# leonsick/depthg

Hardware: AMD Instinct MI355X
Metric: correlation-loss steps/sec at B=32,C=384,28x28 (fwd+bwd, per-GPU batch 32) (higher is better)
Workload: dtype bf16 (feats) / f16 (code) MFMA inputs, f32 accumulate

## Files before the change

### depthg_amd/_lib.py

```python
import ctypes
import os

_HERE = os.path.dirname(os.path.abspath(__file__))
LIB_PATH = os.environ.get("DEPTHG_LIB") or os.path.join(_HERE, "lib", "libdepthg_hip.so")

DG_OUT_COUNT = 9
DG_OUT_TOTAL = 8
DG_VERSION = 118
DG_POINTWISE, DG_ZERO_CLAMP, DG_STABALIZE, DG_DEPTH_TERM, DG_NEED_GRAD, DG_SHARED_COORDS, DG_IDENTITY_GRID, DG_LINE_GRID, \
    DG_EXACT_MASKS, DG_FEATS_UNIT = (1 << i for i in range(10))
DG_LIN_LAYERNORM, DG_LIN_GELU, DG_LIN_IN_BF16, DG_LIN_OUT_BF16 = 1, 2, 4, 8

class CorrDesc(ctypes.Structure):
    _fields_ = [("B", ctypes.c_int32), ("C", ctypes.c_int32), ("D", ctypes.c_int32), ("h", ctypes.c_int32),
                ("w", ctypes.c_int32), ("S", ctypes.c_int32), ("n_neg", ctypes.c_int32),
                ("depth_h", ctypes.c_int32), ("depth_w", ctypes.c_int32), ("flags", ctypes.c_uint32),
                ("shift_intra", ctypes.c_float), ("shift_inter", ctypes.c_float), ("shift_neg", ctypes.c_float),
                ("shift_depth", ctypes.c_float),
                ("w_intra", ctypes.c_float), ("w_inter", ctypes.c_float), ("w_neg", ctypes.c_float),
                ("w_depth", ctypes.c_float), ("code_h", ctypes.c_int32), ("code_w", ctypes.c_int32)]


class AdamSeg(ctypes.Structure):
    _fields_ = [("param", ctypes.c_void_p), ("grad", ctypes.c_void_p), ("exp_avg", ctypes.c_void_p), ("exp_avg_sq", ctypes.c_void_p),
# ... 64 lines not shown
    "dg_crfloss_forward": (_I, [vp, vp] + [i32] * 7 + [vp, i32] + [f32] * 6 + [vp, _SZ, vp, vp]),
    "dg_crfloss_backward": (_I, [vp, _SZ, vp] + [i32] * 6 + [vp, vp, vp]),
    "dg_augalign_workspace_bytes": (_SZ, [i32] * 5),
    "dg_augalign_forward": (_I, [vp] * 3 + [i32] * 7 + [vp, _SZ, vp, vp]),
    "dg_augalign_backward": (_I, [vp, vp, vp, _SZ] + [i32] * 5 + [vp] * 4),
    "dg_recloss_workspace_bytes": (_SZ, [i32] * 5),
    "dg_recloss_forward": (_I, [vp] * 5 + [f32] + [i32] * 5 + [vp, _SZ, vp, vp]),
    "dg_recloss_backward": (_I, [vp] * 5 + [f32, vp, _SZ] + [i32] * 5 + [vp] * 5),
    "dg_adam_step": (_I, [ctypes.POINTER(AdamSeg), i32, ctypes.POINTER(AdamGroup), i32, i32, vp, vp]),
    "dg_attention_workspace_bytes": (_SZ, [i32] * 3),
    "dg_attention_forward": (_I, [vp] + [i32] * 4 + [f32, vp, vp, _SZ, vp]),
    "dg_vit_linear_packed_bytes": (_SZ, [i32] * 2),
    "dg_vit_linear_pack": (_I, [vp, i32, i32, vp, vp]),
    "dg_vit_linear_forward": (_I, [vp, vp, vp, f32, vp, vp, vp, vp] + [i32] * 4 + [vp]),
    "dg_corr_main_kernel_name": (_STR, [cp]),
    "dg_corr_intra_folded": (_I, [cp]),
    "dg_prof_main_span": (_I, [vp]),
    "dg_corr_relaunch_main": (_I, [cp, vp, vp, _SZ, vp]),
}
EXPORTS = list(SIGNATURES)

_lib = None


def load():
    global _lib
    if _lib is not None:
        return _lib
    if not os.path.exists(LIB_PATH):
        raise RuntimeError(
# ... 19 lines not shown
```

### depthg_amd/csrc/dg_api_corr.hip

```cpp
#include "dg_api.h"
#include "dg_corr_args.h"
#include "dg_taps.h"

static unsigned long long* g_prof_span = nullptr;
extern "C" int dg_prof_main_span(void* span) { g_prof_span = static_cast<unsigned long long*>(span); return DG_OK; }

enum class Prep { Small, Dense, General };
enum class Sampler { Plane, ChannelLast };
enum class MainKernel { Small, Corr2, CorrMain };
enum class Depth { None, Job, GsBlocks, GsOwnLaunch };
enum class Hist { Rows, Blobs };
enum class Masks { None, Sampled, DenseRaw, DenseSplit };

struct PairSet {
    int op;
    int neg;
    bool mapped;
    float shift;
    int slot_loss, slot_cd;
    float fin_scale;
    int gidx, csel, dest;
    float factor;
};
struct Operand {
// ... 1 lines not shown
    int cset;
    int map;
};

struct Plan {
    int B, C, D, h, w, hc, wc, S, Sh, P, Ppad, KF, KD, C4, D4, N, T, nops, rf, nrb;
    bool shared, depth, grad, pointwise;
    Prep prep;
    Sampler sampler;
    MainKernel main;
    Masks masks;
    Hist hist;
    bool fold;
    bool half;
    Depth depth_run;
    int nsplit;
    int dep_nrb;
    float lo, hi;
    float shift_depth;
    float inv_numel;
    float grad_f, grad_fn;
    int blob, blob_off_c;
    PairSet ps[DG_MAX_NEG + 2];
    Operand ops[DG_MAX_NEG + 2];
    bool gr_on;
    int gr_nkeys, gr_cpb, gr_blocks_per_image;
    int8_t gr_key[DG_MAX_JOBS], gr_first[DG_MAX_JOBS];
    int32_t gr_nblk[DG_MAX_JOBS];
    size_t nhwc_f[2], nhwc_c[2];
    size_t rows_f[DG_MAX_NEG + 2], rows_c[DG_MAX_NEG + 2];
// ... 147 lines not shown
    p.ticket = take(256);
    const bool xmask = rows && !p.small() && p.grad && plain_zero_clamp && p.Ppad <= 256 && p.rf == 4;
    const bool xmask_dense = (d->flags & DG_EXACT_MASKS) && ident && p.grad && plain_zero_clamp &&
                             p.KF == 384 && p.KD == 96 && p.D <= 80 && p.Ppad >= 160 && p.B <= 64;
    if ((d->flags & DG_EXACT_MASKS) && p.grad && (d->flags & DG_ZERO_CLAMP) && !xmask && !xmask_dense && !p.small())
        return fail(DG_ERR_UNSUPPORTED, "DG_EXACT_MASKS: exact clamp masks exist on small sample grids (always on there) and on the dense "
                                        "identity grid with C <= 384 (padded to 384), D <= 80, P >= 160, B <= 64, zero_clamp without stabalize");
    p.masks = xmask ? Masks::Sampled : (!xmask_dense ? Masks::None : (p.pointwise ? Masks::DenseSplit : Masks::DenseRaw));
    for (int t = 0; t < p.T; ++t) p.maskbits[t] = take(p.has_masks() ? B * (size_t)(p.Ppad / 32) * p.Ppad * 4 : 0);
    p.main = p.small() ? MainKernel::Small
                       : (p.grad && dg_corr2_shape_supported(p.KF, p.KD, p.D, p.lo, p.hi, p.Ppad, p.B) ? MainKernel::Corr2 : MainKernel::CorrMain);
    static const bool fold_on = [] { const char* e = getenv("DG_FOLD_INTRA"); return !(e && e[0] == '0'); }();
    p.fold = fold_on && p.main == MainKernel::Corr2 && p.pointwise && !xmask;
    p.half = p.main == MainKernel::Corr2 && ident && p.N * p.B <= 512 && p.S == p.h && p.S == p.w;
    p.depth_run = (!p.depth || p.small()) ? Depth::None : (!p.grad ? Depth::Job : (p.dense_masks() ? Depth::GsOwnLaunch : Depth::GsBlocks));
    for (int i = 0; i < 2; ++i) p.clo[i] = take(p.masks == Masks::DenseSplit ? B * (size_t)(p.Ppad / 32) * p.KD * 64 : 0);
    p.gr_list = take((size_t)DG_MAX_JOBS * B * DG_GR_CAP * 4);
    p.gr_count = take((size_t)DG_MAX_JOBS * B * 4);
    p.gr_rank = take((size_t)DG_MAX_JOBS * B * 2);
    {
        const bool sg = p.small() && p.grad, two = sg && p.pointwise;
        const size_t gt = B * p.Ppad * p.KD * 4;
        for (int t = 0; t < p.T; ++t) {
            p.dRA2[t] = take(two ? gt : 0);
            p.dRBs[t] = take(sg && p.nsplit == 2 ? gt : 0);
            for (int k = 0; k < 2; ++k) p.dRB2[t][k] = take(two && k < p.nsplit ? gt : 0);
            p.dRBm[t] = take(sg && t >= 2 && (p.pointwise || p.nsplit == 2) ? gt : 0);
        }
        p.part4 = take(p.small() ? (size_t)(p.T + 1) * B * p.nsplit * 16 : 0);
        p.om = take(p.small() ? (size_t)(p.T + 1) * 4 : 0);
// ... 311 lines not shown
        f.ext_inv = c.feat_inv ? c.feat_inv + (size_t)o * p.B * p.P : nullptr;
        f.K = p.C; f.K4 = p.C4; f.Kpad = p.KF; f.is_code = 0; f.h = p.h; f.w = p.w;
        DgGatherJob& k = g.jobs[nj++];
        k.src = p.plane() ? f32(c.ws, p.rows_c[o]) : f32(c.ws, p.nhwc_c[srcsel]); k.coords = c.coords(o); k.srcidx = idx;
        k.blob = c.ws + p.op[o]; k.inv_norm = f32(c.ws, p.inv[o]); k.colpart = f32(c.ws, p.ccolpart[o]);
        k.K = p.D; k.K4 = p.D4; k.Kpad = p.KD; k.is_code = 1; k.h = p.hc; k.w = p.wc;
    }
    g.njobs = nj;
    g.direct = p.plane() ? 1 : 0;
    if (p.masks == Masks::Sampled) cd_mask_args(c, p.rows_c, g.cd);
    g.pre = pre_late;
    DG_HIP(dg_launch_gather(g, p.KF, c.stream));
    return DG_OK;
}

static int fwd_colmeans(Fwd& c) {
    const Plan& p = c.p;
    const DgCorrArgs& a = c.a;
    DgColmeanArgs m;
    memset(&m, 0, sizeof(m));
    m.nops = p.nops; m.B = p.B; m.P = p.P; m.Ppad = p.Ppad; m.KF = p.KF; m.KD = p.KD;
    for (int o = 0; o < p.nops; ++o) {
        m.colpart[o] = p.pointwise ? f32(c.ws, p.colpart[o]) : nullptr; m.bbar[o] = f32(c.ws, p.bbar[o]);
        m.bsplit[o] = reinterpret_cast<__bf16*>(c.ws + p.bsplit[o]);
        m.ngroups[o] = p.Ppad / 32;
        m.ccolpart[o] = f32(c.ws, p.ccolpart[o]); m.csum[o] = f32(c.ws, p.csum[o]);
    }
    m.zero_word = p.depth_in_gs() ? reinterpret_cast<unsigned int*>(c.ws + p.ticket) : nullptr;
    m.zero_words9 = a.wctr;
    if (p.gr_on) {
        m.gr.nh = p.T; m.gr.nkeys = p.gr_nkeys; m.gr.B = p.B;
        for (int t = 0; t < p.T; ++t) { m.gr.sidx[t] = p.map_of(t, c.perms); m.gr.key[t] = p.gr_key[t]; }
        m.gr.list = reinterpret_cast<int32_t*>(c.ws + p.gr_list); m.gr.count = reinterpret_cast<int32_t*>(c.ws + p.gr_count);
        m.gr.rank = reinterpret_cast<int16_t*>(c.ws + p.gr_rank);
    }
    if (p.dense() && p.pointwise) {
        m.dc.code[0] = c.code; m.dc.code[1] = c.code_pos;
        for (int o = 0; o < 2; ++o) { m.dc.blob[o] = c.ws + p.op[o]; m.dc.inv_norm[o] = f32(c.ws, p.inv[o]); m.dc.ccolpart[o] = f32(c.ws, p.ccolpart[o]); }
        m.dc.B = p.B; m.dc.D = p.D; m.dc.KF = p.KF; m.dc.KD = p.KD; m.dc.h = p.h; m.dc.w = p.w; m.dc.P = p.P; m.dc.Ppad = p.Ppad;
        if (p.masks == Masks::DenseSplit) { m.dc.clo[0] = c.ws + p.clo[0]; m.dc.clo[1] = c.ws + p.clo[1]; }
    }
    if (c.split) {
        DgColmeanArgs ms = m;
        ms.zsel = 1; m.zsel = 2;
        DG_HIP(c.side->hand_over(0));
        DG_HIP(dg_launch_colmean(ms, c.side->stream()));
    }
    DG_HIP(dg_launch_colmean(m, c.stream));
    return DG_OK;
}

static int fwd_cd_mask3(Fwd& c) {
    const Plan& p = c.p;
    DgCdMask3Args m;
    memset(&m, 0, sizeof(m));
    m.opR = c.ws + p.op[0]; m.loR = c.ws + p.clo[0];
// ... 97 lines not shown
    if (int rc = make_plan(desc, c.p)) return rc;
    const Plan& p = c.p;
    c.desc = desc; c.feats = orig_feats; c.feats_pos = orig_feats_pos; c.code = orig_code; c.code_pos = orig_code_pos; c.depth = depth;
    c.coords1 = coords1; c.coords2 = coords2; c.perms = perms; c.draw = draw; c.fk = fk; c.feat_inv = feat_inv; c.out = out_scalars;
    c.stream = static_cast<hipStream_t>(stream_);
    if (int rc = fwd_validate(c, workspace, workspace_bytes)) return rc;

    if (p.dense_masks() && split_masks_enabled()) c.side.emplace(c.stream);
    c.split = c.side && static_cast<bool>(*c.side) && p.pointwise;

    if (p.small()) return forward_small(c);
    if (int rc = p.dense() ? fwd_operands_dense(c) : fwd_operands_general(c)) return rc;

    build_corr_jobs(p, c.ws, perms, c.a);

    if (int rc = fwd_colmeans(c)) return rc;
    if (p.masks == Masks::DenseSplit) { if (int rc = fwd_cd_mask3(c)) return rc; }
    if (p.pointwise) { if (int rc = fwd_rowmeans(c)) return rc; }

    if (c.split) DG_HIP(c.side->join());
    if (int rc = launch_main(p, c.a, c.stream)) return rc;

    return fwd_finish(c);
}

extern "C" int dg_corr_forward(const dg_corr_desc* desc, const float* orig_feats, const float* orig_feats_pos,
                               const float* orig_code, const float* orig_code_pos, const float* depth,
                               const float* coords1, const float* coords2, const int64_t* perms,
                               float* out_scalars, void* workspace, size_t workspace_bytes, dg_stream_t stream_) {
    return corr_forward_impl(desc, orig_feats, orig_feats_pos, orig_code, orig_code_pos, depth, coords1, coords2, perms, nullptr,
                             out_scalars, workspace, workspace_bytes, stream_);
}

// ... 231 lines not shown
    return launch_main(p, a, static_cast<hipStream_t>(stream_));
}

extern "C" int dg_corr_intra_folded(const dg_corr_desc* desc) {
    Plan p{};
    if (make_plan(desc, p) != DG_OK) return -1;
    return p.fold ? 1 : 0;
}

extern "C" const char* dg_corr_main_kernel_name(const dg_corr_desc* desc) {
    Plan p{};
    if (make_plan(desc, p) != DG_OK) return nullptr;
    return p.main == MainKernel::Small ? "k_corr_small" : (p.main == MainKernel::Corr2 ? "k_corr2" : "k_corr_main");
}

extern "C" int dg_normalize_split(int32_t B, int32_t C, int32_t h, int32_t w, const float* src, int32_t nchunks, int32_t chunk_c,
                                  float* const* dst, dg_stream_t stream_) {
    if (B < 1 || C < 1 || h < 1 || w < 1 || !src || !dst) return fail(DG_ERR_INVALID, "dg_normalize_split: bad arguments");
    if (nchunks < 1 || nchunks > 16 || chunk_c < 1 || (long long)chunk_c * (nchunks - 1) >= C || (long long)chunk_c * nchunks < C)
        return fail(DG_ERR_INVALID, "dg_normalize_split: %d chunks of %d channels do not tile C=%d (at most 16 chunks)", nchunks, chunk_c, C);
    for (int k = 0; k < nchunks; ++k) if (!dst[k]) return fail(DG_ERR_INVALID, "dg_normalize_split: null destination %d", k);
    DG_HIP(dg_launch_normalize_split(src, B, C, h * w, nchunks, chunk_c, dst, static_cast<hipStream_t>(stream_)));
    return DG_OK;
}
```

### depthg_amd/csrc/dg_corr_args.h

```cpp
#pragma once
#include "dg_device.h"

__host__ __device__ inline int dg_perm32(int pl) {
    int s = pl >> 4, u = (pl >> 3) & 1, hh = (pl >> 2) & 1, v = pl & 3;
    return (2 * s + hh) * 8 + 4 * u + v;
}

#ifndef DG_F_IG
#define DG_F_IG 4
#endif
__host__ __device__ inline int dg_f_off(int q, int g) {
    constexpr int IG = DG_F_IG;
    return ((g / IG) * 32 + q) * (IG * 16) + (((g % IG) ^ ((q / (16 / IG)) % IG)) * 16);
}

struct DgBlob {
    int GF, GD, KD;
    int off_c, off_p, bytes;
    __host__ __device__ DgBlob(int KF, int KD_) : GF(KF / 8), GD(KD_ / 8), KD(KD_) {
        off_c = 32 * GF * 16;
        off_p = off_c + GD * 32 * 16;
        bytes = off_p + 4 * KD * 16;
    }
    __host__ __device__ int f(int q, int g) const { return dg_f_off(q, g); }
// ... 356 lines not shown
    const __bf16* bsplit;
    const int64_t* aidx;
    const int64_t* bidx;
    float* rvec;
    float* rimg;
};
struct DgRowmeanArgs {
    DgRowmeanJob jobs[DG_MAX_NEG + 2];
    int32_t njobs, B, P, Ppad, KF, KD;
    const float* abar;
    char* stash;
    int32_t stash_off;
    const float* cs_part[2];
    float* cs_out[2];
    int32_t ncs;
};

struct DgScatterSrc {
    const float* buf;
    const int64_t* route;
    int32_t gidx;
    int32_t coords_sel;
    float factor;
    int32_t dest;
    int32_t raw;
    const float* dfac;
    int32_t half;
};
#define DG_MAX_SCATTER 48
struct DgScatterArgs {
// ... 81 lines not shown
    const char* opR;
    const char* opS[DG_MAX_NEG + 2];
    const float* rowsR;
    const float* rowsS[DG_MAX_NEG + 2];
    const int64_t* sidx[DG_MAX_NEG + 2];
    unsigned long long* out;
    int32_t count, B, P, Ppad, D, D4, KD, blob_bytes, off_c;
    int32_t nbins;
    float lo, scale;
};
hipError_t dg_launch_cd_hist(const DgCdHistArgs& a, bool rows, hipStream_t s);
hipError_t dg_launch_plane_sample(const DgPlaneArgs& a, hipStream_t s);
hipError_t dg_launch_colmean(const DgColmeanArgs& a, hipStream_t s);
hipError_t dg_launch_prep_dense(const DgDenseArgs& a, hipStream_t s);
hipError_t dg_launch_rowmean(const DgRowmeanArgs& a, hipStream_t s);
hipError_t dg_launch_set_stash(char* blobs, int B, int ntiles, size_t blob_bytes, int off, const float* rvec, int P, int Ppad, hipStream_t s);
hipError_t dg_launch_scatter(const DgScatterArgs& a, hipStream_t s);
hipError_t dg_launch_super_perms(const float* keys, uint64_t seed, unsigned long long* state, int count, int B, int64_t* out, hipStream_t s);
hipError_t dg_launch_pre_general(const struct DgPreArgs& a, hipStream_t s);
bool dg_small_supported(int Ppad, int KD);
hipError_t dg_launch_corr_small(const struct DgSmallArgs& a, hipStream_t s);
hipError_t dg_launch_small_finish(const struct DgSmallArgs& a, hipStream_t s);
hipError_t dg_launch_gather_rows(const struct DgGatherRowsArgs& a, hipStream_t s);
hipError_t dg_launch_rand_coords_state(unsigned long long* state, float* out, int n, hipStream_t s, float keep_p = -1.f);
hipError_t dg_launch_fps(const float* depth, const float* depth_b, int Ba, int B, int H, int W, int h, int w, int S, float factor,
                         float* out_coords, int32_t* out_inds, float* pooled_ws, hipStream_t s);
hipError_t dg_launch_sampled_sumsq(const float* feats, const float* coords, const int64_t* srcidx, float* out, int B, int C, int h, int w, int S, int Sh, int accumulate, hipStream_t s);
hipError_t dg_launch_normalize_split(const float* src, int B, int C, int P, int nchunks, int chunk_c, float* const* dst, hipStream_t s);
```

### depthg_amd/csrc/dg_prep.hip

```cpp
#include "dg_device.h"
#include "dg_corr_args.h"
#include "dg_taps.h"
#include <cstdlib>

__global__ void k_nchw_to_nhwc(const DgTransposeArgs a) {
    __shared__ float t[32][33];
    const int b = blockIdx.z;
    int m = 0, gy = blockIdx.y;
    while (m < a.nmaps - 1 && gy >= (a.K4[m] + 31) / 32) { gy -= (a.K4[m] + 31) / 32; ++m; }
    const float* __restrict__ src = a.src[m];
    float* __restrict__ dst = a.dst[m];
    const int K = a.K[m], K4 = a.K4[m], HW = a.HW[m];
    const int k0 = gy * 32, p0 = blockIdx.x * 32;
    if (p0 >= HW) return;
    const int tx = threadIdx.x, ty = threadIdx.y;
    for (int i = ty; i < 32; i += 8) {
        int k = k0 + i, p = p0 + tx;
        t[i][tx] = (k < K && p < HW) ? src[((size_t)b * K + k) * HW + p] : 0.f;
    }
    __syncthreads();
    for (int i = ty; i < 32; i += 8) {
        int p = p0 + i, k = k0 + tx;
        if (p < HW && k < K4) dst[((size_t)b * HW + p) * K4 + k] = t[tx][i];
    }
// ... 682 lines not shown
        for (int p = a.P + threadIdx.x; p < a.Ppad; p += 256) inv[p] = 0.f;
    if (i >= HW) return;
    const float* src = a.code[o] + (size_t)n * a.D * HW + i;
    float t[4 * UN];
#pragma unroll
    for (int k = 0; k < 4 * UN; ++k) t[k] = k < a.D ? src[(size_t)k * HW] : 0.f;
    float ss[4] = {0.f, 0.f, 0.f, 0.f};
#pragma unroll
    for (int u = 0; u < UN; ++u)
#pragma unroll
        for (int kg = 0; kg < 4; ++kg) ss[kg] = fmaf(t[kg + 4 * u], t[kg + 4 * u], ss[kg]);
    const float tot = ss[0] + ss[1] + ss[2] + ss[3];
    inv[i] = 1.f / fmaxf(sqrtf(tot), DG_EPS_NORM);
}

__device__ __forceinline__ void dense_code_planes(const DgDenseCodeArgs& a, char* xt, int n, int o, int g) {
    const int tid = threadIdx.x, HW = a.h * a.w, nt = a.Ppad / 32, KD = a.KD;
    const DgBlob L(a.KF, a.KD);
    const int nch = min(8, a.D - 8 * g);
    char* const xl = xt + (size_t)a.Ppad * 16;
    const bool want_lo = a.clo[o] != nullptr;
    for (int p = a.P + tid; p < a.Ppad; p += 256) {
        reinterpret_cast<uint4*>(xt)[p] = make_uint4(0u, 0u, 0u, 0u);
        if (want_lo) reinterpret_cast<uint4*>(xl)[p] = make_uint4(0u, 0u, 0u, 0u);
    }
    if (nch <= 0) {
        for (int p = tid; p < a.P; p += 256) {
            reinterpret_cast<uint4*>(xt)[p] = make_uint4(0u, 0u, 0u, 0u);
            if (want_lo) reinterpret_cast<uint4*>(xl)[p] = make_uint4(0u, 0u, 0u, 0u);
        }
    } else {
// ... 19 lines not shown
                for (int c = 0; c < 8; ++c) v[c] = c < nch ? (_Float16)(t[j][c] * iv[j]) : (_Float16)0.f;
                *reinterpret_cast<f16x8*>(xt + pp[j] * 16) = v;
                if (want_lo) {
                    f16x8 l;
#pragma unroll
                    for (int c = 0; c < 8; ++c) l[c] = c < nch ? (_Float16)((t[j][c] * iv[j] - (float)v[c]) * 2048.f) : (_Float16)0.f;
                    *reinterpret_cast<f16x8*>(xl + pp[j] * 16) = l;
                }
            }
        }
    }
    __syncthreads();
    char* blob0 = a.blob[o] + (size_t)n * nt * L.bytes;
    for (int id = tid; id < nt * 32; id += 256) {
        const int tl = id >> 5, qq = id & 31;
        *reinterpret_cast<uint4*>(blob0 + (size_t)tl * L.bytes + L.c(qq, g)) = reinterpret_cast<const uint4*>(xt)[id];
        if (want_lo)
            *reinterpret_cast<uint4*>(a.clo[o] + ((size_t)n * nt + tl) * (KD * 64) + (g * 32 + qq) * 16) = reinterpret_cast<const uint4*>(xl)[id];
    }
    for (int id = tid; id < nt * 32; id += 256) {
        const int tl = id >> 5, cc = (id >> 3) & 3, c = id & 7;
        f16x8 v;
#pragma unroll
        for (int e = 0; e < 8; ++e) {
            const int pl = 16 * (cc >> 1) + 8 * ((e >> 2) & 1) + 4 * (cc & 1) + (e & 3);
            v[e] = *reinterpret_cast<const _Float16*>(xt + (tl * 32 + pl) * 16 + c * 2);
        }
        *reinterpret_cast<f16x8*>(blob0 + (size_t)tl * L.bytes + L.p(8 * g + c, cc)) = v;
    }
    for (int id = tid; id < nt * 8; id += 256) {
        const int tl = id >> 3, c = id & 7;
        float cs = 0.f;
#pragma unroll 8
        for (int qq = 0; qq < 32; ++qq) cs += (float)*reinterpret_cast<const _Float16*>(xt + (tl * 32 + qq) * 16 + c * 2);
        a.ccolpart[o][((size_t)n * nt + tl) * KD + 8 * g + c] = cs;
    }
}


template <int MAXU, int UNC, bool FK = false>
__global__ __launch_bounds__(256) void k_prep_dense(const DgDenseArgs a) {
    extern __shared__ float sl[];
    int bid;
    {
        const int nwg = gridDim.x, orig = blockIdx.x;
        const int q = nwg >> 3, rem = nwg & 7, xcd = orig & 7;
        bid = (xcd < rem ? xcd * (q + 1) : rem * (q + 1) + (xcd - rem) * q) + (orig >> 3);
    }
    const int gx = a.Ppad / 32;
    const int nz = a.depth ? 5 : 4;
// ... 167 lines not shown

hipError_t dg_launch_colmean(const DgColmeanArgs& a, hipStream_t s) {
    int ny = a.gr.nkeys > a.nops ? a.gr.nkeys : a.nops;
    int nz = a.gr.nkeys > 0 ? 3 : 2, smem = 0;
    if (a.dc.B > 0) {
        if (a.nops != 2) return hipErrorInvalidValue;
        ny = max(ny, 2 * (a.dc.KD / 8)); nz = 4; smem = a.dc.Ppad * 16 * ((a.dc.clo[0] || a.dc.clo[1]) ? 2 : 1);
        hipError_t e = dg_set_max_smem(reinterpret_cast<const void*>(k_colmean), smem);
        if (e != hipSuccess) return e;
    }
    hipLaunchKernelGGL(k_colmean, dim3(a.B, ny, nz), dim3(256), smem, s, a);
    return hipGetLastError();
}

#define ROWMEAN_WAVES 4
__global__ __launch_bounds__(64 * ROWMEAN_WAVES) void k_rowmean(const DgRowmeanArgs a) {
    extern __shared__ __attribute__((aligned(16))) char rm_smem[];
    const int tile = blockIdx.x, n = blockIdx.y, tid = threadIdx.x, lane = tid & 63, c = lane & 31, h = lane >> 5;
    const int wid = __builtin_amdgcn_readfirstlane(tid >> 6);
    const int KF = a.KF, nt = a.Ppad / 32;
    if (tile == nt + 1) {
        for (int o = 0; o < a.ncs; ++o) colsum_reduce(a.cs_part[o], n, nt, a.KD, 1.f, a.cs_out[o]);
        return;
    }
    if (tile == nt) {
        float av[12];
#pragma unroll
        for (int j = 0; j < 12; ++j) av[j] = lane + 64 * j < KF ? a.abar[(size_t)n * KF + lane + 64 * j] : 0.f;
        for (int t = wid; t < a.njobs; t += ROWMEAN_WAVES) {
            const DgRowmeanJob& Jt = a.jobs[t];
            const float* bt = Jt.bbar + (size_t)(Jt.bidx ? (int)Jt.bidx[n] : n) * KF;
            float s = 0.f;
#pragma unroll
            for (int j = 0; j < 12; ++j) s = fmaf(av[j], lane + 64 * j < KF ? bt[lane + 64 * j] : 0.f, s);
#pragma unroll
            for (int o = 32; o > 0; o >>= 1) s += __shfl_xor(s, o, 64);
            if (lane == 0) Jt.rimg[n] = s * (float)a.P;
        }
        return;
    }
    const DgBlob L(a.KF, a.KD);
    const int jb = c & 15, lo = c >> 4;
    const bool has = jb < a.njobs;
    const DgRowmeanJob& J = a.jobs[has ? jb : 0];
    const int nb = J.bidx ? (int)J.bidx[n] : n;
    const int nks = KF / 16 / ROWMEAN_WAVES;
    const int pieces = L.off_c / 1024 / ROWMEAN_WAVES;
    const char* fp = a.jobs[0].A + ((size_t)n * nt + tile) * L.bytes + lane * 16;
    const uint32_t dst = lds_addr(rm_smem);
    for (int pc = wid * pieces; pc < (wid + 1) * pieces; ++pc) dma16(fp + pc * 1024, dst + pc * 1024);
    const __bf16* bb = J.bsplit + ((size_t)nb * 2 + lo) * KF + 8 * h;
    f32x16 acc = {};
    asm volatile("s_waitcnt vmcnt(0)" ::: "memory");
    for (int ks0 = wid * nks; ks0 < (wid + 1) * nks; ks0 += 2) {
        bf16x8 af[2], bf[2];
#pragma unroll
        for (int u = 0; u < 2; ++u) {
            const int ks = ks0 + u;
            af[u] = *reinterpret_cast<const bf16x8*>(rm_smem + dg_f_off(c, 2 * ks + h));
            bf[u] = *reinterpret_cast<const bf16x8*>(bb + 16 * ks);
        }
#pragma unroll
        for (int u = 0; u < 2; ++u) {
            bf16x8 b = bf[u];
            if (!has) {
#pragma unroll
                for (int e = 0; e < 8; ++e) b[e] = (__bf16)0.f;
            }
            acc = __builtin_amdgcn_mfma_f32_32x32x16_bf16(af[u], b, acc, 0, 0, 0);
        }
    }
    __syncthreads();
    float* red = reinterpret_cast<float*>(rm_smem);
    if (wid > 0) {
#pragma unroll
        for (int i = 0; i < 16; ++i) red[((wid - 1) * 16 + i) * 64 + lane] = acc[i];
    }
    __syncthreads();
    if (wid != 0) return;
#pragma unroll
    for (int w = 0; w < ROWMEAN_WAVES - 1; ++w)
#pragma unroll
        for (int i = 0; i < 16; ++i) acc[i] += red[(w * 16 + i) * 64 + lane];
#pragma unroll
    for (int i = 0; i < 16; ++i) {
        const float v = acc[i] + __shfl(acc[i], (lane + 16) & 63, 64);
        const int p = tile * 32 + (i & 3) + 8 * (i >> 2) + 4 * h;
        if (has && !lo) J.rvec[(size_t)n * a.Ppad + p] = p < a.P ? v : 0.f;
        if (a.stash && has && !lo && jb == 0) {
            const float x = p < a.P ? -0.5f * v : 0.f;
            const _Float16 xh = (_Float16)x, xl = (_Float16)((x - (float)xh) * 2048.f);
            const uint32_t word = (uint32_t)__builtin_bit_cast(unsigned short, xh) | ((uint32_t)__builtin_bit_cast(unsigned short, xl) << 16);
            *reinterpret_cast<uint32_t*>(a.stash + ((size_t)n * nt + tile) * L.bytes + L.off_c + a.stash_off + (p & 31) * 16) = word;
        }
    }
}
__global__ __launch_bounds__(64) void k_set_stash(char* blobs, size_t blob_bytes, int off, const float* rvec, int ntiles, int P, int Ppad) {
    if (threadIdx.x >= 32) return;
    uint32_t word = 0u;
    if (rvec) {
        const int n = (int)blockIdx.x / ntiles, tile = (int)blockIdx.x - n * ntiles, p = tile * 32 + (int)threadIdx.x;
        const float x = p < P ? -0.5f * rvec[(size_t)n * Ppad + p] : 0.f;
        const _Float16 xh = (_Float16)x, xl = (_Float16)((x - (float)xh) * 2048.f);
        word = (uint32_t)__builtin_bit_cast(unsigned short, xh) | ((uint32_t)__builtin_bit_cast(unsigned short, xl) << 16);
    }
    *reinterpret_cast<uint32_t*>(blobs + (size_t)blockIdx.x * blob_bytes + off + threadIdx.x * 16) = word;
}
hipError_t dg_launch_set_stash(char* blobs, int B, int ntiles, size_t blob_bytes, int off, const float* rvec, int P, int Ppad, hipStream_t s) {
    hipLaunchKernelGGL(k_set_stash, dim3(B * ntiles), dim3(64), 0, s, blobs, blob_bytes, off, rvec, ntiles, P, Ppad);
    return hipGetLastError();
}
// ... 10 lines not shown
```

### depthg_amd/ops.py

```python
import collections
import ctypes
import math
import os

import torch

from . import _lib
from ._lib import CorrDesc


POISON = os.environ.get("DG_POISON", "") not in ("", "0")


def _empty(shape, dtype, device):
    t = torch.empty(shape, dtype=dtype, device=device)
    if POISON and t.numel():
        t.reshape(-1).view(torch.uint8).fill_(0xFF)
    return t


def _ptr(t):
    return ctypes.c_void_p(t.data_ptr()) if t is not None else ctypes.c_void_p(0)


# ... 858 lines not shown
        return self.last()[0]


def corr_intra_folded(desc):
    rc = _lib.load().dg_corr_intra_folded(ctypes.byref(desc))
    if rc < 0:
        _lib.check(-1, "dg_corr_intra_folded")
    return rc == 1


def corr_main_kernel_name(desc):
    name = _lib.load().dg_corr_main_kernel_name(ctypes.byref(desc))
    if name is None:
        _lib.check(-1, "dg_corr_main_kernel_name")
    return name.decode()


HeadPlan = collections.namedtuple("HeadPlan", "dh_route dh_blocks tiles wgrad_pair wgrad_single s2a s1 s2b step_major")
_HEAD_DH_ROUTES = ("TILES", "FUSED")
_HEAD_WGRAD_FORMS = ("DIRECT", "GROUPED", "ONE_PASS")


def head_plan(B, C, D, P):
    out = (ctypes.c_int32 * 9)()
    _lib.check(_lib.load().dg_head_plan_describe(int(B), int(C), int(D), int(P), out), "dg_head_plan_describe")
    v = list(out)
    return HeadPlan(_HEAD_DH_ROUTES[v[0]], v[1], v[2], _HEAD_WGRAD_FORMS[v[3]], _HEAD_WGRAD_FORMS[v[4]], v[5], v[6], v[7], bool(v[8]))


def attention_forward(qkv, heads, scale=None, out=None):
# ... 128 lines not shown
```

### include/depthg_corr.h

```cpp
#ifndef DEPTHG_CORR_H
#define DEPTHG_CORR_H

#include <stddef.h>
#include <stdint.h>

#ifdef __cplusplus
extern "C" {
#endif

#define DG_VERSION 118

#define DG_POINTWISE      (1u << 0)
#define DG_ZERO_CLAMP     (1u << 1)
#define DG_STABALIZE      (1u << 2)
#define DG_DEPTH_TERM     (1u << 3)
#define DG_NEED_GRAD      (1u << 4)
#define DG_SHARED_COORDS  (1u << 5)

#define DG_IDENTITY_GRID  (1u << 6)

#define DG_LINE_GRID      (1u << 7)

#define DG_EXACT_MASKS    (1u << 8)

// ... 242 lines not shown
size_t dg_attention_workspace_bytes(int32_t B, int32_t heads, int32_t N);
int dg_attention_forward(const float* qkv, int32_t B, int32_t N, int32_t heads, int32_t head_dim, float scale, float* out,
                         void* workspace, size_t workspace_bytes, dg_stream_t stream);

#define DG_LIN_LAYERNORM 1
#define DG_LIN_GELU      2
#define DG_LIN_IN_BF16   4
#define DG_LIN_OUT_BF16  8
size_t dg_vit_linear_packed_bytes(int32_t K, int32_t Nout);
int dg_vit_linear_pack(const float* weight, int32_t K, int32_t Nout, void* packed, dg_stream_t stream);
int dg_vit_linear_forward(const void* x, const float* gamma, const float* beta, float eps, const void* packed, const float* bias,
                          const float* residual, void* out, int32_t M, int32_t K, int32_t Nout, int32_t flags, dg_stream_t stream);

const char* dg_corr_main_kernel_name(const dg_corr_desc* desc);

int dg_corr_intra_folded(const dg_corr_desc* desc);

int dg_prof_main_span(void* span);

int dg_corr_relaunch_main(const dg_corr_desc* desc, const int64_t* perms,
                          void* workspace, size_t workspace_bytes, dg_stream_t stream);

#ifdef __cplusplus
}
#endif
#endif
```

Before: 3294.

## Fuse column means, row means, and code planes into one dense means kernel

When the grid is identity, the loss is pointwise, and there are no masks, the separate colmean, rowmean, and dense-code prep launches are replaced by a single k_means_dense launch. Blocks are partitioned by role: row-mean tiles that rebuild the means in LDS from column partials, an image-mean block, code-plane blocks that also write per-channel column sums, and group-list blocks. The goal is to cut launch count and inter-kernel serialization in the forward pass. In exchange, each row-mean block redundantly reduces the column partials, and the fused kernel needs a larger LDS footprint.

```diff
diff --git a/depthg_amd/_lib.py b/depthg_amd/_lib.py
--- a/depthg_amd/_lib.py
+++ b/depthg_amd/_lib.py
@@ -102,6 +102,7 @@
     "dg_vit_linear_pack": (_I, [vp, i32, i32, vp, vp]),
     "dg_vit_linear_forward": (_I, [vp, vp, vp, f32, vp, vp, vp, vp] + [i32] * 4 + [vp]),
     "dg_corr_main_kernel_name": (_STR, [cp]),
+    "dg_corr_means_kernel_names": (_STR, [cp]),
     "dg_corr_intra_folded": (_I, [cp]),
     "dg_prof_main_span": (_I, [vp]),
     "dg_corr_relaunch_main": (_I, [cp, vp, vp, _SZ, vp]),
diff --git a/depthg_amd/csrc/dg_api_corr.hip b/depthg_amd/csrc/dg_api_corr.hip
--- a/depthg_amd/csrc/dg_api_corr.hip
+++ b/depthg_amd/csrc/dg_api_corr.hip
@@ -39,6 +39,7 @@
     bool fold;
     bool half;
     Depth depth_run;
+    bool means_one;
     int nsplit;
     int dep_nrb;
     float lo, hi;
@@ -216,6 +217,7 @@
     p.fold = fold_on && p.main == MainKernel::Corr2 && p.pointwise && !xmask;
     p.half = p.main == MainKernel::Corr2 && ident && p.N * p.B <= 512 && p.S == p.h && p.S == p.w;
     p.depth_run = (!p.depth || p.small()) ? Depth::None : (!p.grad ? Depth::Job : (p.dense_masks() ? Depth::GsOwnLaunch : Depth::GsBlocks));
+    p.means_one = ident && p.pointwise && p.masks == Masks::None;
     for (int i = 0; i < 2; ++i) p.clo[i] = take(p.masks == Masks::DenseSplit ? B * (size_t)(p.Ppad / 32) * p.KD * 64 : 0);
     p.gr_list = take((size_t)DG_MAX_JOBS * B * DG_GR_CAP * 4);
     p.gr_count = take((size_t)DG_MAX_JOBS * B * 4);
@@ -557,6 +559,42 @@
     return DG_OK;
 }
 
+static void group_args(const Fwd& c, DgGroupArgs& gr) {
+    const Plan& p = c.p;
+    if (!p.gr_on) return;
+    gr.nh = p.T; gr.nkeys = p.gr_nkeys; gr.B = p.B;
+    for (int t = 0; t < p.T; ++t) { gr.sidx[t] = p.map_of(t, c.perms); gr.key[t] = p.gr_key[t]; }
+    gr.list = reinterpret_cast<int32_t*>(c.ws + p.gr_list); gr.count = reinterpret_cast<int32_t*>(c.ws + p.gr_count);
+    gr.rank = reinterpret_cast<int16_t*>(c.ws + p.gr_rank);
+}
+static void dense_code_args(const Fwd& c, DgDenseCodeArgs& dc) {
+    const Plan& p = c.p;
+    dc.code[0] = c.code; dc.code[1] = c.code_pos;
+    for (int o = 0; o < 2; ++o) { dc.blob[o] = c.ws + p.op[o]; dc.inv_norm[o] = f32(c.ws, p.inv[o]); dc.ccolpart[o] = f32(c.ws, p.ccolpart[o]); }
+    dc.B = p.B; dc.D = p.D; dc.KF = p.KF; dc.KD = p.KD; dc.h = p.h; dc.w = p.w; dc.P = p.P; dc.Ppad = p.Ppad;
+    if (p.masks == Masks::DenseSplit) { dc.clo[0] = c.ws + p.clo[0]; dc.clo[1] = c.ws + p.clo[1]; }
+}
+
+static int fwd_means_dense(Fwd& c) {
+    const Plan& p = c.p;
+    DgMeansDenseArgs m;
+    memset(&m, 0, sizeof(m));
+    m.B = p.B; m.P = p.P; m.Ppad = p.Ppad; m.KF = p.KF; m.KD = p.KD; m.njobs = p.T;
+    m.A = c.ws + p.op[0]; m.acolpart = f32(c.ws, p.colpart[0]);
+    for (int t = 0; t < p.T; ++t) {
+        m.jobs[t].colpart = f32(c.ws, p.colpart[p.ps[t].op]); m.jobs[t].bidx = p.map_of(t, c.perms);
+        m.jobs[t].rvec = f32(c.ws, p.rvec[t]); m.jobs[t].rimg = f32(c.ws, p.rimg[t]);
+    }
+    for (int o = 0; o < 2; ++o) m.csum[o] = f32(c.ws, p.csum[o]);
+    if (p.fold) { m.stash = c.ws + p.op[0]; m.stash_off = FOLD_STASH_OFF; }
+    m.zero_word = p.depth_in_gs() ? reinterpret_cast<unsigned int*>(c.ws + p.ticket) : nullptr;
+    m.zero_words9 = c.a.wctr;
+    group_args(c, m.gr);
+    dense_code_args(c, m.dc);
+    DG_HIP(dg_launch_means_dense(m, c.stream));
+    return DG_OK;
+}
+
 static int fwd_colmeans(Fwd& c) {
     const Plan& p = c.p;
     const DgCorrArgs& a = c.a;
@@ -571,18 +609,8 @@
     }
     m.zero_word = p.depth_in_gs() ? reinterpret_cast<unsigned int*>(c.ws + p.ticket) : nullptr;
     m.zero_words9 = a.wctr;
-    if (p.gr_on) {
-        m.gr.nh = p.T; m.gr.nkeys = p.gr_nkeys; m.gr.B = p.B;
-        for (int t = 0; t < p.T; ++t) { m.gr.sidx[t] = p.map_of(t, c.perms); m.gr.key[t] = p.gr_key[t]; }
-        m.gr.list = reinterpret_cast<int32_t*>(c.ws + p.gr_list); m.gr.count = reinterpret_cast<int32_t*>(c.ws + p.gr_count);
-        m.gr.rank = reinterpret_cast<int16_t*>(c.ws + p.gr_rank);
-    }
-    if (p.dense() && p.pointwise) {
-        m.dc.code[0] = c.code; m.dc.code[1] = c.code_pos;
-        for (int o = 0; o < 2; ++o) { m.dc.blob[o] = c.ws + p.op[o]; m.dc.inv_norm[o] = f32(c.ws, p.inv[o]); m.dc.ccolpart[o] = f32(c.ws, p.ccolpart[o]); }
-        m.dc.B = p.B; m.dc.D = p.D; m.dc.KF = p.KF; m.dc.KD = p.KD; m.dc.h = p.h; m.dc.w = p.w; m.dc.P = p.P; m.dc.Ppad = p.Ppad;
-        if (p.masks == Masks::DenseSplit) { m.dc.clo[0] = c.ws + p.clo[0]; m.dc.clo[1] = c.ws + p.clo[1]; }
-    }
+    group_args(c, m.gr);
+    if (p.dense() && p.pointwise) dense_code_args(c, m.dc);
     if (c.split) {
         DgColmeanArgs ms = m;
         ms.zsel = 1; m.zsel = 2;
@@ -710,9 +738,13 @@
 
     build_corr_jobs(p, c.ws, perms, c.a);
 
-    if (int rc = fwd_colmeans(c)) return rc;
-    if (p.masks == Masks::DenseSplit) { if (int rc = fwd_cd_mask3(c)) return rc; }
-    if (p.pointwise) { if (int rc = fwd_rowmeans(c)) return rc; }
+    if (p.means_one) {
+        if (int rc = fwd_means_dense(c)) return rc;
+    } else {
+        if (int rc = fwd_colmeans(c)) return rc;
+        if (p.masks == Masks::DenseSplit) { if (int rc = fwd_cd_mask3(c)) return rc; }
+        if (p.pointwise) { if (int rc = fwd_rowmeans(c)) return rc; }
+    }
 
     if (c.split) DG_HIP(c.side->join());
     if (int rc = launch_main(p, c.a, c.stream)) return rc;
@@ -974,6 +1006,13 @@
     return p.main == MainKernel::Small ? "k_corr_small" : (p.main == MainKernel::Corr2 ? "k_corr2" : "k_corr_main");
 }
 
+extern "C" const char* dg_corr_means_kernel_names(const dg_corr_desc* desc) {
+    Plan p{};
+    if (make_plan(desc, p) != DG_OK) return nullptr;
+    if (p.small()) return "";
+    return p.means_one ? "k_means_dense" : (p.pointwise ? "k_colmean,k_rowmean" : "k_colmean");
+}
+
 extern "C" int dg_normalize_split(int32_t B, int32_t C, int32_t h, int32_t w, const float* src, int32_t nchunks, int32_t chunk_c,
                                   float* const* dst, dg_stream_t stream_) {
     if (B < 1 || C < 1 || h < 1 || w < 1 || !src || !dst) return fail(DG_ERR_INVALID, "dg_normalize_split: bad arguments");
diff --git a/depthg_amd/csrc/dg_corr_args.h b/depthg_amd/csrc/dg_corr_args.h
--- a/depthg_amd/csrc/dg_corr_args.h
+++ b/depthg_amd/csrc/dg_corr_args.h
@@ -394,6 +394,27 @@
     const float* cs_part[2];
     float* cs_out[2];
     int32_t ncs;
+};
+
+struct DgMeansJob {
+    const float* colpart;
+    const int64_t* bidx;
+    float* rvec;
+    float* rimg;
+};
+struct DgMeansDenseArgs {
+    DgMeansJob jobs[DG_MAX_NEG + 2];
+    const char* A;
+    const float* acolpart;
+    char* stash;
+    int32_t stash_off;
+    float* csum[2];
+    int32_t njobs, B, P, Ppad, KF, KD;
+    int32_t run;
+    unsigned int* zero_word;
+    unsigned int* zero_words9;
+    DgGroupArgs gr;
+    DgDenseCodeArgs dc;
 };
 
 struct DgScatterSrc {
@@ -505,6 +526,7 @@
 hipError_t dg_launch_colmean(const DgColmeanArgs& a, hipStream_t s);
 hipError_t dg_launch_prep_dense(const DgDenseArgs& a, hipStream_t s);
 hipError_t dg_launch_rowmean(const DgRowmeanArgs& a, hipStream_t s);
+hipError_t dg_launch_means_dense(const DgMeansDenseArgs& a, hipStream_t s);
 hipError_t dg_launch_set_stash(char* blobs, int B, int ntiles, size_t blob_bytes, int off, const float* rvec, int P, int Ppad, hipStream_t s);
 hipError_t dg_launch_scatter(const DgScatterArgs& a, hipStream_t s);
 hipError_t dg_launch_super_perms(const float* keys, uint64_t seed, unsigned long long* state, int count, int B, int64_t* out, hipStream_t s);
diff --git a/depthg_amd/csrc/dg_prep.hip b/depthg_amd/csrc/dg_prep.hip
--- a/depthg_amd/csrc/dg_prep.hip
+++ b/depthg_amd/csrc/dg_prep.hip
@@ -720,7 +720,7 @@
     inv[i] = 1.f / fmaxf(sqrtf(tot), DG_EPS_NORM);
 }
 
-__device__ __forceinline__ void dense_code_planes(const DgDenseCodeArgs& a, char* xt, int n, int o, int g) {
+__device__ __forceinline__ void dense_code_planes(const DgDenseCodeArgs& a, char* xt, int n, int o, int g, bool own_c = true, float* csum = nullptr) {
     const int tid = threadIdx.x, HW = a.h * a.w, nt = a.Ppad / 32, KD = a.KD;
     const DgBlob L(a.KF, a.KD);
     const int nch = min(8, a.D - 8 * g);
@@ -770,7 +770,7 @@
     char* blob0 = a.blob[o] + (size_t)n * nt * L.bytes;
     for (int id = tid; id < nt * 32; id += 256) {
         const int tl = id >> 5, qq = id & 31;
-        *reinterpret_cast<uint4*>(blob0 + (size_t)tl * L.bytes + L.c(qq, g)) = reinterpret_cast<const uint4*>(xt)[id];
+        if (own_c) *reinterpret_cast<uint4*>(blob0 + (size_t)tl * L.bytes + L.c(qq, g)) = reinterpret_cast<const uint4*>(xt)[id];
         if (want_lo)
             *reinterpret_cast<uint4*>(a.clo[o] + ((size_t)n * nt + tl) * (KD * 64) + (g * 32 + qq) * 16) = reinterpret_cast<const uint4*>(xl)[id];
     }
@@ -790,6 +790,15 @@
 #pragma unroll 8
         for (int qq = 0; qq < 32; ++qq) cs += (float)*reinterpret_cast<const _Float16*>(xt + (tl * 32 + qq) * 16 + c * 2);
         a.ccolpart[o][((size_t)n * nt + tl) * KD + 8 * g + c] = cs;
+        if (csum) reinterpret_cast<float*>(xt + (size_t)a.Ppad * 16)[id] = cs;
+    }
+    if (!csum) return;
+    __syncthreads();
+    if (tid < 8) {
+        const float* cl = reinterpret_cast<const float*>(xt + (size_t)a.Ppad * 16) + tid;
+        float s = 0.f;
+        for (int tl = 0; tl < nt; ++tl) s += cl[tl * 8];
+        csum[(size_t)n * KD + 8 * g + tid] = s * 1.f;
     }
 }
 
@@ -987,6 +996,68 @@
 }
 
 #define ROWMEAN_WAVES 4
+template <bool MERGED, class Args>
+__device__ __forceinline__ void rowmean_tile(const Args& a, char* rm_smem, const char* ftile, const __bf16* bb, int tile, int n) {
+    const int tid = threadIdx.x, lane = tid & 63, c = lane & 31, h = lane >> 5;
+    const int wid = __builtin_amdgcn_readfirstlane(tid >> 6);
+    const int KF = a.KF, nt = a.Ppad / 32;
+    const DgBlob L(a.KF, a.KD);
+    const int jb = c & 15, lo = c >> 4;
+    const bool has = jb < a.njobs;
+    const auto& J = a.jobs[has ? jb : 0];
+    const int nks = KF / 16 / ROWMEAN_WAVES;
+    const int pieces = L.off_c / 1024 / ROWMEAN_WAVES;
+    const char* fp = ftile + lane * 16;
+    const uint32_t dst = lds_addr(rm_smem);
+    for (int pc = wid * pieces; pc < (wid + 1) * pieces; ++pc) dma16(fp + pc * 1024, dst + pc * 1024);
+    f32x16 acc = {};
+    asm volatile("s_waitcnt vmcnt(0)" ::: "memory");
+    for (int ks0 = wid * nks; ks0 < (wid + 1) * nks; ks0 += 2) {
+        bf16x8 af[2], bf[2];
+#pragma unroll
+        for (int u = 0; u < 2; ++u) {
+            const int ks = ks0 + u;
+            af[u] = *reinterpret_cast<const bf16x8*>(rm_smem + dg_f_off(c, 2 * ks + h));
+            bf[u] = *reinterpret_cast<const bf16x8*>(bb + 16 * ks);
+        }
+#pragma unroll
+        for (int u = 0; u < 2; ++u) {
+            bf16x8 b = bf[u];
+            if (!has) {
+#pragma unroll
+                for (int e = 0; e < 8; ++e) b[e] = (__bf16)0.f;
+            }
+            acc = __builtin_amdgcn_mfma_f32_32x32x16_bf16(af[u], b, acc, 0, 0, 0);
+        }
+    }
+    __syncthreads();
+    float* red = reinterpret_cast<float*>(rm_smem);
+    if (wid > 0) {
+#pragma unroll
+        for (int i = 0; i < 16; ++i) red[((wid - 1) * 16 + i) * 64 + lane] = acc[i];
+    }
+    __syncthreads();
+    if (wid != 0) return;
+#pragma unroll
+    for (int w = 0; w < ROWMEAN_WAVES - 1; ++w)
+#pragma unroll
+        for (int i = 0; i < 16; ++i) acc[i] += red[(w * 16 + i) * 64 + lane];
+#pragma unroll
+    for (int i = 0; i < 16; ++i) {
+        const float v = acc[i] + __shfl(acc[i], (lane + 16) & 63, 64);
+        const int p = tile * 32 + (i & 3) + 8 * (i >> 2) + 4 * h;
+        if (has && !lo) J.rvec[(size_t)n * a.Ppad + p] = p < a.P ? v : 0.f;
+        if (a.stash && has && !lo && jb == 0) {
+            const float x = p < a.P ? -0.5f * v : 0.f;
+            const _Float16 xh = (_Float16)x, xl = (_Float16)((x - (float)xh) * 2048.f);
+            const uint32_t word = (uint32_t)__builtin_bit_cast(unsigned short, xh) | ((uint32_t)__builtin_bit_cast(unsigned short, xl) << 16);
+            char* w = a.stash + ((size_t)n * nt + tile) * L.bytes + L.off_c + a.stash_off + (p & 31) * 16;
+            if (MERGED) *reinterpret_cast<uint4*>(w) = make_uint4(word, 0u, 0u, 0u);
+            else *reinterpret_cast<uint32_t*>(w) = word;
+        }
+    }
+}
+
 __global__ __launch_bounds__(64 * ROWMEAN_WAVES) void k_rowmean(const DgRowmeanArgs a) {
     extern __shared__ __attribute__((aligned(16))) char rm_smem[];
     const int tile = blockIdx.x, n = blockIdx.y, tid = threadIdx.x, lane = tid & 63, c = lane & 31, h = lane >> 5;
@@ -1014,60 +1085,129 @@
     }
     const DgBlob L(a.KF, a.KD);
     const int jb = c & 15, lo = c >> 4;
-    const bool has = jb < a.njobs;
-    const DgRowmeanJob& J = a.jobs[has ? jb : 0];
+    const DgRowmeanJob& J = a.jobs[jb < a.njobs ? jb : 0];
     const int nb = J.bidx ? (int)J.bidx[n] : n;
-    const int nks = KF / 16 / ROWMEAN_WAVES;
-    const int pieces = L.off_c / 1024 / ROWMEAN_WAVES;
-    const char* fp = a.jobs[0].A + ((size_t)n * nt + tile) * L.bytes + lane * 16;
-    const uint32_t dst = lds_addr(rm_smem);
-    for (int pc = wid * pieces; pc < (wid + 1) * pieces; ++pc) dma16(fp + pc * 1024, dst + pc * 1024);
-    const __bf16* bb = J.bsplit + ((size_t)nb * 2 + lo) * KF + 8 * h;
-    f32x16 acc = {};
-    asm volatile("s_waitcnt vmcnt(0)" ::: "memory");
-    for (int ks0 = wid * nks; ks0 < (wid + 1) * nks; ks0 += 2) {
-        bf16x8 af[2], bf[2];
-#pragma unroll
-        for (int u = 0; u < 2; ++u) {
-            const int ks = ks0 + u;
-            af[u] = *reinterpret_cast<const bf16x8*>(rm_smem + dg_f_off(c, 2 * ks + h));
-            bf[u] = *reinterpret_cast<const bf16x8*>(bb + 16 * ks);
-        }
-#pragma unroll
-        for (int u = 0; u < 2; ++u) {
-            bf16x8 b = bf[u];
-            if (!has) {
-#pragma unroll
-                for (int e = 0; e < 8; ++e) b[e] = (__bf16)0.f;
-            }
-            acc = __builtin_amdgcn_mfma_f32_32x32x16_bf16(af[u], b, acc, 0, 0, 0);
-        }
-    }
-    __syncthreads();
-    float* red = reinterpret_cast<float*>(rm_smem);
-    if (wid > 0) {
-#pragma unroll
-        for (int i = 0; i < 16; ++i) red[((wid - 1) * 16 + i) * 64 + lane] = acc[i];
-    }
-    __syncthreads();
-    if (wid != 0) return;
-#pragma unroll
-    for (int w = 0; w < ROWMEAN_WAVES - 1; ++w)
-#pragma unroll
-        for (int i = 0; i < 16; ++i) acc[i] += red[(w * 16 + i) * 64 + lane];
-#pragma unroll
-    for (int i = 0; i < 16; ++i) {
-        const float v = acc[i] + __shfl(acc[i], (lane + 16) & 63, 64);
-        const int p = tile * 32 + (i & 3) + 8 * (i >> 2) + 4 * h;
-        if (has && !lo) J.rvec[(size_t)n * a.Ppad + p] = p < a.P ? v : 0.f;
-        if (a.stash && has && !lo && jb == 0) {
-            const float x = p < a.P ? -0.5f * v : 0.f;
-            const _Float16 xh = (_Float16)x, xl = (_Float16)((x - (float)xh) * 2048.f);
-            const uint32_t word = (uint32_t)__builtin_bit_cast(unsigned short, xh) | ((uint32_t)__builtin_bit_cast(unsigned short, xl) << 16);
-            *reinterpret_cast<uint32_t*>(a.stash + ((size_t)n * nt + tile) * L.bytes + L.off_c + a.stash_off + (p & 31) * 16) = word;
-        }
-    }
-}
+    rowmean_tile<false>(a, rm_smem, a.jobs[0].A + ((size_t)n * nt + tile) * L.bytes, J.bsplit + ((size_t)nb * 2 + lo) * KF + 8 * h, tile, n);
+}
+
+#define MEANS_RUN 2
+#define MEANS_BROW(KF) ((KF) * 2 + 16)
+template <bool F32>
+__device__ __forceinline__ void means_to_lds(const DgMeansDenseArgs& a, int n, float* mf, char* bs) {
+    const int KF = a.KF, KF4 = KF / 4, nt = a.Ppad / 32, nvec = a.njobs + (F32 ? 1 : 0);
+    const float scale = 1.f / (float)a.P;
+    for (int id = threadIdx.x; id < nvec * KF4; id += 256) {
+        const int j = id / KF4, k4 = id - j * KF4;
+        const bool isa = j == a.njobs;
+        const DgMeansJob& J = a.jobs[isa ? 0 : j];
+        const float* part = isa ? a.acolpart : J.colpart;
+        const int nb = (!isa && J.bidx) ? (int)J.bidx[n] : n;
+        const f32x4* cp = reinterpret_cast<const f32x4*>(part + (size_t)nb * nt * KF) + k4;
+        f32x4 s = {0.f, 0.f, 0.f, 0.f};
+        for (int t = 0; t < nt; t += 8) {
+            f32x4 v[8];
+#pragma unroll
+            for (int u = 0; u < 8; ++u) v[u] = t + u < nt ? cp[(size_t)(t + u) * KF4] : f32x4{0.f, 0.f, 0.f, 0.f};
+#pragma unroll
+            for (int u = 0; u < 8; ++u) if (t + u < nt) s += v[u];
+        }
+#pragma unroll
+        for (int e = 0; e < 4; ++e) s[e] = dg_mul_rn(s[e], scale);
+        if (F32) {
+            *reinterpret_cast<f32x4*>(mf + (size_t)j * KF + 4 * k4) = s;
+        } else {
+            bf16x4 hi, lo;
+#pragma unroll
+            for (int e = 0; e < 4; ++e) { hi[e] = (__bf16)s[e]; lo[e] = (__bf16)(s[e] - (float)hi[e]); }
+            *reinterpret_cast<bf16x4*>(bs + (size_t)(2 * j) * MEANS_BROW(KF) + 8 * k4) = hi;
+            *reinterpret_cast<bf16x4*>(bs + (size_t)(2 * j + 1) * MEANS_BROW(KF) + 8 * k4) = lo;
+        }
+    }
+}
+
+__global__ __launch_bounds__(256) void k_means_dense(const DgMeansDenseArgs a) {
+    extern __shared__ __attribute__((aligned(16))) char md_smem[];
+    int bid;
+    {
+        const int nwg = gridDim.x, orig = blockIdx.x;
+        const int q = nwg >> 3, rem = nwg & 7, xcd = orig & 7;
+        bid = (xcd < rem ? xcd * (q + 1) : rem * (q + 1) + (xcd - rem) * q) + (orig >> 3);
+    }
+    const int tid = threadIdx.x, lane = tid & 63, nt = a.Ppad / 32, KF = a.KF;
+    const int wid = __builtin_amdgcn_readfirstlane(tid >> 6);
+    const int nrb = (nt + a.run - 1) / a.run, GD = a.dc.KD / 8;
+    const int per = nrb + 1 + 2 * GD + a.gr.nkeys;
+    const int n = bid / per;
+    int r = bid - n * per;
+    if (bid == 0) {
+        if (a.zero_word && tid == 0) *a.zero_word = 0u;
+        if (a.zero_words9 && tid < 9) a.zero_words9[tid] = 0u;
+    }
+    if (r < nrb) {
+        const int stage = max(32 * (KF / 8) * 16, (ROWMEAN_WAVES - 1) * 16 * 64 * 4);
+        char* bs = md_smem + stage;
+        means_to_lds<false>(a, n, nullptr, bs);
+        __syncthreads();
+        const DgBlob L(a.KF, a.KD);
+        const int c = lane & 31, h = lane >> 5, jb = c & 15, lo = c >> 4;
+        const __bf16* bb = reinterpret_cast<const __bf16*>(bs + (size_t)(2 * (jb < a.njobs ? jb : 0) + lo) * MEANS_BROW(KF)) + 8 * h;
+        const int t1 = min(nt, (r + 1) * a.run);
+        for (int tile = r * a.run; tile < t1; ++tile) {
+            rowmean_tile<true>(a, md_smem, a.A + ((size_t)n * nt + tile) * L.bytes, bb, tile, n);
+            __syncthreads();
+        }
+        return;
+    }
+    r -= nrb;
+    if (r == 0) {
+        float* mf = reinterpret_cast<float*>(md_smem);
+        means_to_lds<true>(a, n, mf, nullptr);
+        __syncthreads();
+        float av[12];
+#pragma unroll
+        for (int j = 0; j < 12; ++j) av[j] = lane + 64 * j < KF ? mf[(size_t)a.njobs * KF + lane + 64 * j] : 0.f;
+        for (int t = wid; t < a.njobs; t += ROWMEAN_WAVES) {
+            const float* bt = mf + (size_t)t * KF;
+            float s = 0.f;
+#pragma unroll
+            for (int j = 0; j < 12; ++j) s = fmaf(av[j], lane + 64 * j < KF ? bt[lane + 64 * j] : 0.f, s);
+#pragma unroll
+            for (int o = 32; o > 0; o >>= 1) s += __shfl_xor(s, o, 64);
+            if (lane == 0) a.jobs[t].rimg[n] = s * (float)a.P;
+        }
+        return;
+    }
+    r -= 1;
+    if (r < 2 * GD) {
+        const int o = r / GD, g = r - o * GD;
+        const bool stash_granule = a.stash && o == 0 && g * 512 == a.stash_off;
+        dense_code_planes(a.dc, md_smem, n, o, g, !stash_granule, a.csum[o]);
+        return;
+    }
+    r -= 2 * GD;
+    if (tid < 64) dg_group_lists(a.gr, n, r, tid);
+}
+
+hipError_t dg_launch_means_dense(const DgMeansDenseArgs& a0, hipStream_t s) {
+    DgMeansDenseArgs a = a0;
+    const int nt = a.Ppad / 32;
+    if (a.njobs < 1 || a.njobs > DG_MAX_NEG + 2 || a.KF > 768 || a.KF % 64 || a.dc.B != a.B || a.dc.clo[0] || a.dc.clo[1] || !a.csum[0] || !a.csum[1])
+        return hipErrorInvalidValue;
+    if (a.stash && (a.stash_off % 512 || a.stash_off / 512 >= a.KD / 8 || a.stash_off / 512 * 8 < a.dc.D)) return hipErrorInvalidValue;
+    if (a.run <= 0) a.run = MEANS_RUN;
+#ifdef DG_DEVTOOLS
+    if (const char* e = getenv("DG_MEANS_RUN")) a.run = atoi(e) > 0 ? atoi(e) : nt;
+#endif
+    a.run = min(a.run, nt);
+    const int stage = max(32 * (a.KF / 8) * 16, (ROWMEAN_WAVES - 1) * 16 * 64 * 4);
+    const int smem = max(max(stage + 2 * a.njobs * MEANS_BROW(a.KF), (a.njobs + 1) * a.KF * 4), a.Ppad * 16 + nt * 8 * 4);
+    hipError_t e = dg_set_max_smem(reinterpret_cast<const void*>(k_means_dense), smem);
+    if (e != hipSuccess) return e;
+    const int per = (nt + a.run - 1) / a.run + 1 + 2 * (a.KD / 8) + a.gr.nkeys;
+    hipLaunchKernelGGL(k_means_dense, dim3(a.B * per), dim3(256), smem, s, a);
+    return hipGetLastError();
+}
+
 __global__ __launch_bounds__(64) void k_set_stash(char* blobs, size_t blob_bytes, int off, const float* rvec, int ntiles, int P, int Ppad) {
     if (threadIdx.x >= 32) return;
     uint32_t word = 0u;
diff --git a/depthg_amd/ops.py b/depthg_amd/ops.py
--- a/depthg_amd/ops.py
+++ b/depthg_amd/ops.py
@@ -896,6 +896,13 @@
     if name is None:
         _lib.check(-1, "dg_corr_main_kernel_name")
     return name.decode()
+
+
+def corr_means_kernel_names(desc):
+    names = _lib.load().dg_corr_means_kernel_names(ctypes.byref(desc))
+    if names is None:
+        _lib.check(-1, "dg_corr_means_kernel_names")
+    return tuple(n for n in names.decode().split(",") if n)
 
 
 HeadPlan = collections.namedtuple("HeadPlan", "dh_route dh_blocks tiles wgrad_pair wgrad_single s2a s1 s2b step_major")
diff --git a/include/depthg_corr.h b/include/depthg_corr.h
--- a/include/depthg_corr.h
+++ b/include/depthg_corr.h
@@ -280,6 +280,8 @@
 
 const char* dg_corr_main_kernel_name(const dg_corr_desc* desc);
 
+const char* dg_corr_means_kernel_names(const dg_corr_desc* desc);
+
 int dg_corr_intra_folded(const dg_corr_desc* desc);
 
 int dg_prof_main_span(void* span);
```

Result: slower. 3253 (-1.2%).
